# dyollb/segmantic

Hardware: AMD Instinct MI355X
Metric: 3D UNet train voxels/s on 128^3 bf16 (higher is better)
Workload: dtype bf16

## Files before the change

### include/segmi.h

```cpp
#ifndef SEGMI_H_
#define SEGMI_H_

#include <stddef.h>
#include <stdint.h>

#ifdef __cplusplus
extern "C" {
#endif

#define SEGMI_VERSION 1

enum { SEGMI_F32 = 0, SEGMI_BF16 = 1, SEGMI_F16 = 2 };
enum { SEGMI_OK = 0, SEGMI_EINVAL = -1, SEGMI_EUNSUPPORTED = -2, SEGMI_ELAUNCH = -3,
       SEGMI_EDATA = -4  };

typedef struct segmi_act {
  void* data;
  int32_t n, d, h, w;
  int32_t c;
  int32_t ld;
} segmi_act;

int segmi_version(void);
const char* segmi_last_error(void);
// ... 82 lines not shown
                               const void* packed, const float* bias, const float* prelu_alpha,
                               int act_channels, int ksize, int stride,
                               const float* bias_b , float* stats_partials ,
                               const segmi_bn_fin* stats_fin , void* stream);
int segmi_conv3d_fwd_pair(int dtype, const segmi_act* in, const segmi_act* out_a, const float* w_a,
                          const float* bias_a, const float* prelu_alpha_a, float* stats_partials_a,
                          const segmi_act* out_b, const float* w_b, const float* bias_b, int stride,
                          const segmi_bn_fin* stats_fin_a ,
                          const segmi_windows* windows ,
                          void* stream);

int segmi_convT3d_stats_rows(int dtype, const segmi_act* in, const segmi_act* out);
int segmi_convT3d_fwd(int dtype, const segmi_act* in, const segmi_act* out, const void* packed,
                      const float* w_src, const float* bias, const float* prelu_alpha,
                      const segmi_act* residual, float* stats_partials,
                      const segmi_bn_fin* stats_fin , void* stream);

int64_t segmi_conv3d_wgrad_workspace(int dtype, const segmi_act* x, const segmi_act* dy,
                                     int ksize, int stride, int cus);
int segmi_conv3d_wgrad(int dtype, const segmi_act* x, const segmi_act* dy, float* dw,
                       float* db, int ksize, int stride, void* workspace,
                       const segmi_in_affine* in_tf , int cus, void* stream);
int segmi_wgrad_cus(int cus);
int segmi_bias_grad(int dtype, const segmi_act* dy, float* db, void* workspace, void* stream);

int segmi_bn_stats_rows(const segmi_act* x);
int segmi_bn_stats(int dtype, const segmi_act* x, float* stats_partials, void* stream);
int segmi_bn_finalize(const float* stats_partials, int rows, int c, double count,
                      const float* gamma, const float* beta, float* running_mean,
                      float* running_var, float momentum, float eps, float* mean,
                      float* invstd, float* scale, float* shift, void* stream);
int segmi_bn_eval_affine(int c, const float* gamma, const float* beta,
                         const float* running_mean, const float* running_var, float eps,
                         float* scale, float* shift, void* stream);
int segmi_bn_act_fwd(int dtype, const segmi_act* x, const segmi_act* y, const float* scale,
                     const float* shift, const float* prelu_alpha, const segmi_act* residual,
                     float dropout_p, uint32_t dropout_seed, void* stream);
int segmi_bn_act_bwd_rows(const segmi_act* x);
int segmi_bn_act_bwd_reduce(int dtype, const segmi_act* dy, const segmi_act* x,
                            const float* mean, const float* invstd, const float* gamma,
                            const float* beta, const float* prelu_alpha, float* red_partials,
                            float dropout_p, uint32_t dropout_seed,
                            const segmi_bn_bwd_fin* fin , void* stream);
int segmi_bn_act_bwd_finalize(const float* red_partials, int rows, int c, double count,
                              const float* gamma, const float* invstd, float* dgamma,
                              float* dbeta, float* dalpha, float* coef, void* stream);
// ... 338 lines not shown
```

### segmantic_amd/_lib.py

```python
from __future__ import annotations

import ctypes as C
import os
from pathlib import Path

import torch

SEGMI_F32 = 0
SEGMI_BF16 = 1
SEGMI_F16 = 2

_LIB_PATH = Path(__file__).resolve().parent / "csrc" / "libsegmi.so"


class Act(C.Structure):

    _fields_ = [("data", C.c_void_p), ("n", C.c_int32), ("d", C.c_int32), ("h", C.c_int32),
                ("w", C.c_int32), ("c", C.c_int32), ("ld", C.c_int32)]


class WpackDesc(C.Structure):

    _fields_ = [("w_src", C.c_void_p), ("scale", C.c_void_p), ("packed", C.c_void_p),
                ("kind", C.c_int32), ("cin_k", C.c_int32), ("cout_k", C.c_int32),
# ... 50 lines not shown
    "segmi_last_error": (C.c_char_p, []),
    "segmi_stream_create_cumask": (_i, [_i, C.POINTER(C.c_void_p)]),
    "segmi_stream_destroy": (_i, [_P]),
    "segmi_wpack_bytes": (_i64, [_i, _i, _i, _i, _i]),
    "segmi_wpack": (_i, [_i, _i, _P, _P, _i, _i, _i, _P, _P]),
    "segmi_wpack_batch": (_i, [_i, C.POINTER(WpackDesc), _i, _P, _i, _P]),
    "segmi_conv3d_stats_rows": (_i, [_i, _AP, _AP, _i, _i]),
    "segmi_conv3d_in_affine_ok": (_i, [_i, _AP, _AP, _i, _i]),
    "segmi_conv3d_fwd_kernel_name": (C.c_char_p, [_i, _AP, _AP, _i, _i]),
    "segmi_conv3d_split_act_ok": (_i, [_i, _AP, _AP, _i, _i]),
    "segmi_conv3d_fwd_split_act": (_i, [_i, _AP, _AP, _P, _P, _P, _i, _i, _i, _P, _P, C.POINTER(BnFin), _P]),
    "segmi_conv3d_fwd": (_i, [_i, _AP, _AP, _P, _P, _i, _P, _P, _AP, _P, _i, _i, C.POINTER(InAffine),
                              C.POINTER(BnBwdSums), C.POINTER(BnFin), _P]),
    "segmi_conv3d_bn_bwd_sums_ok": (_i, [_i, _AP, _AP, _i, _i]),
    "segmi_dectop_ok": (_i, [_i, _AP, _AP]),
    "segmi_dectop_fwd": (_i, [_i, _AP, _AP, _P, _P, _P, _i, _P, _P, _P]),
    "segmi_conv3d_pair_ok": (_i, [_i, _AP, _AP, _AP]),
    "segmi_conv3d_fwd_pair": (_i, [_i, _AP, _AP, _P, _P, _P, _P, _AP, _P, _P, _i, C.POINTER(BnFin),
                                   C.POINTER(Windows), _P]),
    "segmi_convT3d_stats_rows": (_i, [_i, _AP, _AP]),
    "segmi_convT3d_fwd": (_i, [_i, _AP, _AP, _P, _P, _P, _P, _AP, _P, C.POINTER(BnFin), _P]),
    "segmi_conv3d_wgrad_workspace": (_i64, [_i, _AP, _AP, _i, _i, _i]),
    "segmi_conv3d_wgrad": (_i, [_i, _AP, _AP, _P, _P, _i, _i, _P, C.POINTER(InAffine), _i, _P]),
    "segmi_bias_grad": (_i, [_i, _AP, _P, _P, _P]),
    "segmi_bn_stats_rows": (_i, [_AP]),
    "segmi_bn_stats": (_i, [_i, _AP, _P, _P]),
    "segmi_bn_finalize": (_i, [_P, _i, _i, _d, _P, _P, _P, _P, _f, _f, _P, _P, _P, _P, _P]),
    "segmi_bn_eval_affine": (_i, [_i, _P, _P, _P, _P, _f, _P, _P, _P]),
    "segmi_bn_act_fwd": (_i, [_i, _AP, _AP, _P, _P, _P, _AP, _f, C.c_uint32, _P]),
    "segmi_bn_act_bwd_rows": (_i, [_AP]),
    "segmi_bn_act_bwd_reduce": (_i, [_i, _AP, _AP, _P, _P, _P, _P, _P, _P, _f, C.c_uint32,
                                     C.POINTER(BnBwdFin), _P]),
    "segmi_bn_act_bwd_finalize": (_i, [_P, _i, _i, _d, _P, _P, _P, _P, _P, _P, _P]),
    "segmi_bn_act_bwd_fused_ok": (_i, [_i, _AP, _AP, _AP]),
    "segmi_bn_act_bwd_fused_rows": (_i, [_AP]),
    "segmi_bn_act_bwd_fused": (_i, [_i, _AP, _AP, _AP, _P, _P, _P, _P, _P, _P, C.POINTER(BnBwdFin), _i, _P]),
    "segmi_bn_act_bwd_fused_wgs": (_i, [_i, _AP, _i]),
    "segmi_fused_timeouts": (C.c_uint, [_i]),
    "segmi_fused_test_hook": (_i, [C.c_uint, _i]),
    "segmi_bn_act_bwd_apply": (_i, [_i, _AP, _AP, _AP, _P, _P, _P, _P, _P, _P, _f, C.c_uint32, _P]),
    "segmi_bn_act_bwd_apply_conv_ok": (_i, [_i, _AP, _AP, _AP, _AP]),
    "segmi_bn_act_bwd_apply_conv": (_i, [_i, _AP, _AP, _AP, _P, _P, _P, _P, _P, _P, _AP, _P, _P]),
    "segmi_wgrad_cus": (_i, [_i]),
    "segmi_add": (_i, [_i, _AP, _AP, _AP, _P]),
    "segmi_cast_copy": (_i, [_i, _AP, _i, _AP, _P]),
    "segmi_nchw_to_ndhwc": (_i, [_P, _i, _AP, _P]),
# ... 151 lines not shown
```

### segmantic_amd/csrc/conv_small.hip

```cpp
#include "conv_shared.h"

namespace segmi {

struct SmallConvParams {
  const void* in;
  void* out;
  const float* w;
  const float* bias;
  const float* alpha;
  const void* res;
  float* stats;
  int N, Di, Hi, Wi, Do, Ho, Wo, Cout, ldi, ldo, ldr;
  int tz, ty, tx;
  void* out2;
  const float* w2;
  const float* bias2;
  int ldo2;
  int vec;
  int nwin;
  int wsy;
  int64_t wsz;
  int64_t woff[32];
  int fin_on;
  FinTail ft;
// ... 378 lines not shown
        }
      }
    }
  }

  __syncthreads();
  float* red = reinterpret_cast<float*>(smem);
#pragma unroll
  for (int nt = 0; nt < NTL; ++nt)
    *reinterpret_cast<f32x4*>(red + ((wave * NTL + nt) * 64 + lane) * 4) = acc[nt];
  __syncthreads();
  float* slab = p.partials + (int64_t)blockIdx.x * p.Cout * COMBOS;
  for (int o = tid; o < 16 * COMBOS; o += 256) {
    const int co = o / COMBOS, cb = o % COMBOS;
    const int nt = cb / 16, n16 = cb % 16;
    const int src = (nt * 64 + (co >> 2) * 16 + n16) * 4 + (co & 3);
    float sacc = 0.f;
#pragma unroll
    for (int w = 0; w < 4; ++w) sacc += red[w * NTL * 256 + src];
    slab[(int64_t)(co0 + co) * COMBOS + cb] = sacc;
  }
}

bool conv_small_ok(int cin, int cout, int ksize) {
  return ksize == 3 && cin >= 1 && cin <= 4 && (cout == 16 || cout == 32);
}

int conv_small_fwd_rows(const segmi_act* out) {
  return out->n * cdiv(out->d, 4) * cdiv(out->h, 8) * cdiv(out->w, 16);
}

template <typename T, int S, int CIN, bool PAIR>
static int launch_small_fwd_k(SmallConvParams p, hipStream_t st) {
  constexpr int HD = 3 * S + 3, HH = 7 * S + 3, HW = 15 * S + 3, XW = (HW + 6) / 4 * 4;
  constexpr int stage = CIN * HD * HH * XW * (int)sizeof(T);
  constexpr int lds0 = stage > 4 * 2 * 16 * 4 ? stage : 4 * 2 * 16 * 4;
  dim3 grid((unsigned)(p.N * p.tz * p.ty * p.tx), (unsigned)(p.Cout / 16));
  p.fin_on = p.fin_on && p.stats;
  const int lds = (int)fin_tail_arm(p, grid, 256, 2 * p.Cout, lds0);
  static int attr_set = 0;
  if (lds > 64 * 1024 && attr_set < lds) {
    (void)hipFuncSetAttribute((const void*)conv_small_fwd_kernel<T, S, CIN, PAIR>,
                              hipFuncAttributeMaxDynamicSharedMemorySize, lds);
    attr_set = lds;
  }
  hipLaunchKernelGGL((conv_small_fwd_kernel<T, S, CIN, PAIR>), grid, 256, lds, st, p);
// ... 62 lines not shown
  switch (cin) {
    case 1: return launch_small_wgrad<T, S, 1>(p, grid, st);
    case 2: return launch_small_wgrad<T, S, 2>(p, grid, st);
    case 3: return launch_small_wgrad<T, S, 3>(p, grid, st);
    default: return launch_small_wgrad<T, S, 4>(p, grid, st);
  }
}

int conv_small_wgrad(int dtype, const segmi_act* x, const segmi_act* dy, float* partials,
                     int stride, hipStream_t st) {
  SmallWgradParams p{};
  p.x = x->data; p.dy = dy->data; p.partials = partials;
  p.N = x->n; p.Dx = x->d; p.Hx = x->h; p.Wx = x->w; p.Dy = dy->d; p.Hy = dy->h; p.Wy = dy->w;
  p.Cout = dy->c; p.ldx = x->ld; p.ldy = dy->ld;
  p.tz = cdiv(dy->d, 2); p.ty = cdiv(dy->h, 8); p.tx = cdiv(dy->w, 16);
  p.ntiles = dy->n * p.tz * p.ty * p.tx;
  const int grid = conv_small_wgrad_slabs(dy);
#define SMALL_WGRAD(T) \
  return stride == 2 ? launch_small_wgrad_cin<T, 2>(p, x->c, grid, st) : launch_small_wgrad_cin<T, 1>(p, x->c, grid, st)
  SEGMI_BY_DTYPE(dtype, SMALL_WGRAD);
#undef SMALL_WGRAD
}

}
```

### segmantic_amd/csrc/wgrad.hip

```cpp
#include "wgrad_impl.h"
#include "reduce_fin.h"

#include <atomic>
namespace segmi {
static inline int clamp_cus(int n) {
  n = n / 8 * 8;
  return n < 8 ? 8 : (n > 256 ? 256 : n);
}
int wgrad_cus(int cus) {
  static const int env = [] {
    const char* e = getenv("SEGMI_WGRAD_CUS");
    return e ? clamp_cus(atoi(e)) : 0;
  }();
  if (env) return env;
  return cus > 0 ? clamp_cus(cus) : 256;
}
}
namespace segmi {

int wgrad_mfma_f32(const WgradParams& p, int ksize, int stride, int ct, int gx, hipStream_t st);
int wgrad_mfma_bf16(const WgradParams& p, int ksize, int stride, int ct, int gx, hipStream_t st);
int wgrad_mfma_f16(const WgradParams& p, int ksize, int stride, int ct, int gx, hipStream_t st);
int bn_stats_launch(int dtype, const segmi_act* x, float* partials, hipStream_t st, const BiasFin* bias_fin = nullptr);
int bn_stats_rows_for(const segmi_act* x);
bool conv_small_ok(int cin, int cout, int ksize);
int conv_small_wgrad_slabs(const segmi_act* dy);
int conv_small_wgrad(int dtype, const segmi_act* x, const segmi_act* dy, float* partials,
                     int stride, hipStream_t st);

struct WgDirectParams {
  const void* x;
  const void* dy;
  float* partials;
  int N, Dx, Hx, Wx, Dy, Hy, Wy, Cin, Cout, ldx, ldy, ks, stride;
  int64_t nvox;
  int chunk;
};

template <typename T>
__global__ __launch_bounds__(256) void wgrad_direct_kernel(WgDirectParams p) {
  const int nt = p.ks * p.ks * p.ks, pad = (p.ks - 1) / 2;
  const int nout = p.Cout * p.Cin * nt;
  const T* x = (const T*)p.x;
  const T* dy = (const T*)p.dy;
  for (int o = threadIdx.x; o < nout; o += 256) {
    const int tap = o % nt;
    const int ci = (o / nt) % p.Cin;
    const int co = o / (nt * p.Cin);
    const int kd = tap / (p.ks * p.ks), kh = (tap / p.ks) % p.ks, kw = tap % p.ks;
    float acc = 0.f;
    for (int64_t c0 = (int64_t)blockIdx.x * p.chunk; c0 < p.nvox; c0 += (int64_t)gridDim.x * p.chunk) {
      const int64_t c1 = c0 + p.chunk < p.nvox ? c0 + p.chunk : p.nvox;
      for (int64_t v = c0; v < c1; ++v) {
        int64_t t = v;
        const int ox = t % p.Wy; t /= p.Wy;
        const int oy = t % p.Hy; t /= p.Hy;
        const int oz = t % p.Dy;
        const int n = t / p.Dy;
        const int z = oz * p.stride - pad + kd, y = oy * p.stride - pad + kh,
                  xx = ox * p.stride - pad + kw;
        if ((unsigned)z >= (unsigned)p.Dx || (unsigned)y >= (unsigned)p.Hx ||
            (unsigned)xx >= (unsigned)p.Wx) continue;
        const float a = Elem<T>::ld(dy + v * p.ldy + co);
        const float b = Elem<T>::ld(x + ((((int64_t)n * p.Dx + z) * p.Hx + y) * p.Wx + xx) * p.ldx + ci);
        acc = fmaf(a, b, acc);
      }
    }
    p.partials[(int64_t)blockIdx.x * nout + o] = acc;
  }
}

constexpr int kSlabGroups = 16;
__global__ void slab_reduce_kernel(const float* __restrict__ partials, int nslab, int64_t n,
                                   float* __restrict__ out) {
  const int per = (nslab + gridDim.y - 1) / gridDim.y;
  const int b0 = blockIdx.y * per;
  const int b1 = b0 + per < nslab ? b0 + per : nslab;
  for (int64_t e = blockIdx.x * 256ll + threadIdx.x; e < n; e += (int64_t)gridDim.x * 256) {
    double a0 = 0.0, a1 = 0.0, a2 = 0.0, a3 = 0.0;
    int b = b0;
    for (; b + 3 < b1; b += 4) {
      a0 += (double)partials[(int64_t)b * n + e];
      a1 += (double)partials[(int64_t)(b + 1) * n + e];
      a2 += (double)partials[(int64_t)(b + 2) * n + e];
      a3 += (double)partials[(int64_t)(b + 3) * n + e];
    }
    for (; b < b1; ++b) a0 += (double)partials[(int64_t)b * n + e];
    out[(int64_t)blockIdx.y * n + e] = (float)((a0 + a1) + (a2 + a3));
  }
}

__global__ __launch_bounds__(1024) void slab_reduce_fused_kernel(const float* __restrict__ partials, int nslab,
                                                                 int64_t n, float* __restrict__ out) {
  __shared__ float gs[kSlabGroups][64];
  const int g = threadIdx.x >> 6, lane = threadIdx.x & 63;
  const int per = (nslab + kSlabGroups - 1) / kSlabGroups;
  const int b0 = g * per;
  const int b1 = b0 + per < nslab ? b0 + per : nslab;
  for (int64_t e0 = blockIdx.x * 64ll; e0 < n; e0 += (int64_t)gridDim.x * 64) {
    const int64_t e = e0 + lane;
    double a0 = 0.0, a1 = 0.0, a2 = 0.0, a3 = 0.0;
    if (e < n) {
      int b = b0;
      for (; b + 3 < b1; b += 4) {
        a0 += (double)partials[(int64_t)b * n + e];
        a1 += (double)partials[(int64_t)(b + 1) * n + e];
        a2 += (double)partials[(int64_t)(b + 2) * n + e];
        a3 += (double)partials[(int64_t)(b + 3) * n + e];
      }
      for (; b < b1; ++b) a0 += (double)partials[(int64_t)b * n + e];
    }
    gs[g][lane] = (float)((a0 + a1) + (a2 + a3));
    __syncthreads();
    if (g == 0 && e < n) {
      double c0 = 0.0, c1 = 0.0, c2 = 0.0, c3 = 0.0;
#pragma unroll
      for (int b = 0; b < kSlabGroups; b += 4) {
        c0 += (double)gs[b][lane];
        c1 += (double)gs[b + 1][lane];
        c2 += (double)gs[b + 2][lane];
        c3 += (double)gs[b + 3][lane];
      }
      out[e] = (float)((c0 + c1) + (c2 + c3));
    }
    __syncthreads();
  }
}


static inline bool aligned_rows(const segmi_act* a, int dtype) {
  const int es = dtype_size(dtype);
  return a->ld % (16 / es) == 0 && ((uintptr_t)a->data % 16) == 0;
}
static inline bool wg_mfma_ok(int dtype, const segmi_act* x, const segmi_act* dy, int ksize) {
  return x->c % 16 == 0 && dy->c % 16 == 0 && aligned_rows(x, dtype) && aligned_rows(dy, dtype) &&
         (ksize == 3 || ksize == 1);
}
static inline bool wg_small_ok(int dtype, const segmi_act* x, const segmi_act* dy, int ksize) {
  const int es = dtype_size(dtype);
  (void)es;
  return conv_small_ok(x->c, dy->c, ksize) && aligned_rows(dy, dtype);
}
static inline int wg_direct_blocks(const segmi_act* dy) {
  const int64_t b = cdiv64(act_voxels(dy), 512);
  return (int)(b > 1024 ? 1024 : b);
}
// ... 100 lines not shown
    p.nvox = act_voxels(dy); p.chunk = 512;
#define WG_DIRECT(T) hipLaunchKernelGGL(wgrad_direct_kernel<T>, slabs, 256, 0, st, p)
    SEGMI_BY_DTYPE(dtype, WG_DIRECT);
#undef WG_DIRECT
    SEGMI_LAUNCH_CHECK("conv3d_wgrad(direct)");
  }
  const int rb = grid_1d(nout, 2048);
  float* gsum = (float*)((char*)workspace + align256((int64_t)slabs * nout * 4));
  if (slabs > 2 * kSlabGroups) {
    const int fb = (int)(cdiv64(nout, 64) > 4096 ? 4096 : cdiv64(nout, 64));
    hipLaunchKernelGGL(slab_reduce_fused_kernel, dim3(fb), 1024, 0, st, (const float*)partials, slabs, nout, dw);
  } else {
    hipLaunchKernelGGL(slab_reduce_kernel, dim3(rb, 1), 256, 0, st, (const float*)partials, slabs,
                       nout, dw);
  }
  SEGMI_LAUNCH_CHECK("conv3d_wgrad(reduce)");
  if (db) {
    float* bws = (float*)((char*)gsum + align256((int64_t)kSlabGroups * nout * 4));
    return segmi_bias_grad(dtype, dy, db, bws, stream);
  }
  return SEGMI_OK;
}

}
```

### segmantic_amd/ops.py

```python
from __future__ import annotations

import ctypes as C
import math
from typing import Optional, Sequence

import numpy as np
import torch

from . import _lib
from ._lib import SEGMI_BF16, SEGMI_F16, SEGMI_F32, Act, BnBwdFin, BnBwdSums, BnFin, InAffine, Windows, check, lib

_DT = {torch.float32: SEGMI_F32, torch.bfloat16: SEGMI_BF16, torch.float16: SEGMI_F16}


def dtype_code(t: torch.Tensor) -> int:
    try:
        return _DT[t.dtype]
    except KeyError:
        raise TypeError(f"unsupported activation dtype {t.dtype} (float32 / bfloat16 / float16 only)")


def _stream() -> int:
    return torch.cuda.current_stream().cuda_stream

# ... 251 lines not shown
    return int(lib.segmi_convT3d_stats_rows(dtype_code(x), C.byref(ax), C.byref(ay)))


def convT3d_fwd(x, y, packed, w_src, bias, prelu_alpha=None, residual=None, stats=None,
                stats_fin=None) -> None:
    ax, ay = act(x), act(y)
    ar = act(residual) if residual is not None else None
    check(lib.segmi_convT3d_fwd(dtype_code(x), C.byref(ax), C.byref(ay), _ptr(packed),
                                _ptr(w_src), _ptr(bias), _ptr(prelu_alpha), _ref(ar),
                                _ptr(stats), _bn_fin(stats_fin), _stream()), "convT3d_fwd")


def conv3d_wgrad_workspace(x, dy, ksize, stride, cus: int = 0) -> int:
    ax, ay = act(x), act(dy)
    return int(lib.segmi_conv3d_wgrad_workspace(dtype_code(x), C.byref(ax), C.byref(ay), ksize,
                                                stride, int(cus)))


def conv3d_wgrad(x, dy, dw, db, ksize, stride, workspace, in_tf=None, cus: int = 0) -> None:
    ax, ay = act(x), act(dy)
    check(lib.segmi_conv3d_wgrad(dtype_code(x), C.byref(ax), C.byref(ay), _ptr(dw), _ptr(db),
                                 ksize, stride, _ptr(workspace), _in_affine(in_tf), int(cus), _stream()),
          "conv3d_wgrad")


def bias_grad(dy, db, workspace) -> None:
    ay = act(dy)
    check(lib.segmi_bias_grad(dtype_code(dy), C.byref(ay), _ptr(db), _ptr(workspace),
                              _stream()), "bias_grad")


def bn_stats_rows(x) -> int:
    ax = act(x)
    return int(lib.segmi_bn_stats_rows(C.byref(ax)))


def bn_stats(x, partials) -> None:
    ax = act(x)
    check(lib.segmi_bn_stats(dtype_code(x), C.byref(ax), _ptr(partials), _stream()), "bn_stats")


def bn_finalize(partials, rows, c, count, gamma, beta, running_mean, running_var, momentum,
                eps, mean, invstd, scale, shift) -> None:
    check(lib.segmi_bn_finalize(_ptr(partials), rows, c, float(count), _ptr(gamma), _ptr(beta),
                                _ptr(running_mean), _ptr(running_var), momentum, eps,
                                _ptr(mean), _ptr(invstd), _ptr(scale), _ptr(shift), _stream()),
# ... 1667 lines not shown
```

### segmantic_amd/seg/unet.py

```python
from __future__ import annotations

import math
import os
from typing import Dict, List, Optional, Sequence, Tuple

import torch
import torch.nn as nn

from .. import ops
from . import streams

_HALF = (torch.bfloat16, torch.float16)


class _Box(nn.Module):
    """Name-space node: holds children / parameters, computes nothing."""


def _conv_params(cin: int, cout: int, k: int, dims: int, transposed: bool) -> _Box:
    m = _Box()
    shape = ((cin, cout) if transposed else (cout, cin)) + (k,) * dims
    w = torch.empty(shape)
    nn.init.kaiming_uniform_(w, a=math.sqrt(5))
    fan_in = shape[1] * k ** dims
# ... 579 lines not shown
        if self._carry_open and conv in self._carry_convs:
            self._carried.append((conv, x, dy, need_bias, in_tf))
            return
        main = torch.cuda.current_stream()
        side = self._side_stream() if self.overlap_wgrad else None
        if side is not None:
            ev = torch.cuda.Event()
            ev.record(main)
            side.wait_event(ev)
        cus = self.wgrad_cus_overlap if side is not None else 0
        with torch.cuda.stream(side) if side is not None else _NullCtx():
            if conv.transposed:
                nbytes = ops.conv3d_wgrad_workspace(dy, x, 3, 2, cus)
                ws = self._scratch_buf("wgrad", nbytes)
                self._timed(conv.prefix + ":wgrad", ops.conv3d_wgrad, dy, x, conv.gw, None, 3, 2, ws, cus=cus)
                if need_bias:
                    ops.bias_grad(dy, conv.gb, ws)
            else:
                nbytes = ops.conv3d_wgrad_workspace(x, dy, conv.k, conv.stride, cus)
                ws = self._scratch_buf("wgrad", nbytes)
                self._timed(conv.prefix + ":wgrad", ops.conv3d_wgrad, x, dy, conv.gw,
                            conv.gb if need_bias else None, conv.k, conv.stride, ws, in_tf=in_tf, cus=cus)

    def _bsum_ok(self, conv: _Conv, dy, dx, bn: Optional["_BN"]) -> bool:
        return (bn is not None and self.fuse_bn_bwd and self.dtype in _HALF and self.dropout_p <= 0.0
                and not conv.transposed and conv.stride == 1 and conv.k == 3 and conv.mfma
                and conv.cout == 16
                and ops.conv3d_bn_bwd_sums_ok(dy, dx, 3, 1))

    def _dgrad(self, conv: _Conv, dy, dx, residual=None, bsum=None):
        if bsum is not None:
            bn, x_raw = bsum
            rows = ops.conv3d_stats_rows(dy, dx, conv.k, 1)
            part = self._fstat(rows, bn.c)
            self._timed(conv.prefix + ":dgrad", ops.conv3d_fwd, dy, dx, conv.dgrad_pack(), conv.w, 1,
                        None, conv.k, 1, residual=residual,
                        bn_bwd=(x_raw, bn.mean, bn.invstd, bn.gamma, bn.beta, bn.alpha, part),
                        bn_bwd_fin=self._bwd_fin(bn, x_raw))
            return rows
        if conv.transposed:
            ops.conv3d_fwd(dy, dx, conv.dgrad_pack(), conv.w, 0, None, 3, 2, residual=residual)
        elif conv.stride == 2:
            ops.convT3d_fwd(dy, dx, conv.dgrad_pack(), conv.w, None, residual=residual)
        else:
            self._timed(conv.prefix + ":dgrad", ops.conv3d_fwd, dy, dx, conv.dgrad_pack(), conv.w, 1,
                        None, conv.k, 1, residual=residual)
# ... 53 lines not shown
                self._timed(conv.prefix + ":fwd", ops.conv3d_fwd_split_act, x, m, conv.pair_pack(), conv.b, None,
                            conv.cout, conv.k, conv.stride, bias_b=ru["res"].b, stats=stats,
                            stats_fin=self._stats_fin(bn, r))
                saved[f"in{i}"] = cur
                saved[f"r{i}"] = r
                nconv = ru["units"][i + 1][0]
                if self._tf_ok(r, r, nconv) and nconv.cin == conv.cout and nconv.cout == conv.cout:
                    in_tf = (bn.scale, bn.shift, bn.alpha)
                    cur = r
                else:
                    a = self._buf(f"{pre}.a{i}", (n, d, h, w, conv.cout))
                    ops.bn_act_fwd(r, a, bn.scale, bn.shift, bn.alpha, dropout=bn.drop())
                    cur = a
                continue
            if i == 0 and paired:
                r = self._buf(f"{pre}.r{i}", (n, d, h, w, conv.cout))
                rows = ops.conv3d_stats_rows(x, r, conv.k, conv.stride)
                stats = self._fstat(rows, conv.cout)
                rc = ru["res"]
                self._timed(conv.prefix + ":fwd", ops.conv3d_fwd_pair, x, r, conv.w, conv.b, out,
                            rc.w, rc.b, conv.stride, stats_a=stats, stats_fin_a=self._stats_fin(bn, r))
                saved[f"in{i}"] = cur
                saved[f"r{i}"] = r
                nconv = ru["units"][i + 1][0]
                if self._tf_ok(r, r, nconv) and nconv.cin == conv.cout and nconv.cout == conv.cout:
                    in_tf = (bn.scale, bn.shift, bn.alpha)
                    cur = r
                else:
                    a = self._buf(f"{pre}.a{i}", (n, d, h, w, conv.cout))
                    ops.bn_act_fwd(r, a, bn.scale, bn.shift, bn.alpha, dropout=bn.drop())
                    cur = a
                continue
            if bn is None:
                self._timed(conv.prefix + ":fwd", ops.conv3d_fwd, cur, out, conv.fwd_pack(), conv.w,
                            0, conv.b, conv.k, conv.stride, residual=resid, in_tf=in_tf)
                saved[f"in{i}"] = cur
                saved[f"tf{i}"] = in_tf
                break
            r = self._buf(f"{pre}.r{i}", (n, d, h, w, conv.cout))
            self._conv_train(conv, cur, r, bn, in_tf=in_tf)
            saved[f"in{i}"] = cur
            saved[f"r{i}"] = r
            saved[f"tf{i}"] = in_tf
            in_tf = None
            if last:
                ops.bn_act_fwd(r, out, bn.scale, bn.shift, bn.alpha, residual=resid, dropout=bn.drop())
            else:
                nconv = ru["units"][i + 1][0]
                if self._tf_ok(r, r, nconv) and nconv.cin == conv.cout and nconv.cout == conv.cout:
                    in_tf = (bn.scale, bn.shift, bn.alpha)
                    cur = r
                else:
                    a = self._buf(f"{pre}.a{i}", (n, d, h, w, conv.cout))
                    ops.bn_act_fwd(r, a, bn.scale, bn.shift, bn.alpha, dropout=bn.drop())
                    cur = a
        self._saved[pre] = saved

    def _ru_bwd(self, ru, dout, dx=None, extra=None, dx_bn=None):
        pre = ru["prefix"]
        sv = self._saved[pre]
        x = sv["x"]
        nun = len(ru["units"])
        rc = ru["res"]
        if rc is not None and dx is not None:
            self._dgrad(rc, dout, dx, residual=extra)
        g = dout
        g_rows = 0
        for i in range(nun - 1, -1, -1):
            conv, bn = ru["units"][i]
            xin = sv[f"in{i}"]
            if bn is not None:
                r = sv[f"r{i}"]
                dr = self._buf(f"{pre}.dr{i}", r.shape)
                self._bn_bwd(bn, g, r, dr, sums_rows=g_rows)
            else:
                dr = g
            g_rows = 0
            self._wgrad(conv, xin, dr, need_bias=bn is None and conv is not self._top_bias_conv,
                        in_tf=sv.get(f"tf{i}"))
            if i > 0:
                da = self._buf(f"{pre}.da{i - 1}", xin.shape)
                pbn = ru["units"][i - 1][1]
                if self._bsum_ok(conv, dr, da, pbn):
                    g_rows = self._dgrad(conv, dr, da, bsum=(pbn, sv[f"r{i - 1}"]))
                else:
                    self._dgrad(conv, dr, da)
                g = da
            else:
                first_dr = dr
        if rc is not None:
            self._wgrad(rc, x, dout)
        self._grads_ready(self.param_offsets[f"model.{pre}.conv.unit0.conv.weight"][0])
        if dx is None:
            return 0
        conv0 = ru["units"][0][0]
        bsum = dx_bn if dx_bn is not None and self._bsum_ok(conv0, first_dr, dx, dx_bn[0]) else None
        if rc is not None:
            return self._dgrad(conv0, first_dr, dx, residual=dx, bsum=bsum) or 0
        if extra is not None:
            ops.add(dout, extra, dx)
            return self._dgrad(conv0, first_dr, dx, residual=dx, bsum=bsum) or 0
        return self._dgrad(conv0, first_dr, dx, residual=dout, bsum=bsum) or 0

    def _ru_fwd_eval(self, ru, x, out):
        pre = ru["prefix"]
        n, d, h, w = self._down_shape(x.shape, ru["stride"])
        paired = False
        merged = None
        if ru["res"] is not None:
            rc = ru["res"]
            paired = self._pair_ok(ru, x, out, f"{pre}.ea0", (n, d, h, w))
            if isinstance(x, ops.WindowBatch) and not paired:
                raise RuntimeError("window views need the first-layer pair kernel (window_views_ok said yes?)")
# ... 315 lines not shown
```

Before: 3.646 billion.

## Fuse first-unit BN backward apply with paired main and residual weight-gradient kernels

```diff
diff --git a/include/segmi.h b/include/segmi.h
--- a/include/segmi.h
+++ b/include/segmi.h
@@ -128,6 +128,14 @@
                        float* db, int ksize, int stride, void* workspace,
                        const segmi_in_affine* in_tf , int cus, void* stream);
 int segmi_wgrad_cus(int cus);
+int segmi_conv3d_wgrad_pair_ok(int dtype, const segmi_act* x, const segmi_act* g, const segmi_act* x_raw,
+                               const segmi_act* dy_b, int stride);
+int64_t segmi_conv3d_wgrad_pair_workspace(int dtype, const segmi_act* x, const segmi_act* dy_b);
+int segmi_conv3d_wgrad_pair(int dtype, const segmi_act* x, const segmi_act* g, const segmi_act* x_raw,
+                            const float* mean, const float* invstd, const float* gamma ,
+                            const float* beta , const float* prelu_alpha ,
+                            const float* coef, const segmi_act* dy_b, float* dw_a, float* dw_b,
+                            float* db_b , int stride, void* workspace, void* stream);
 int segmi_bias_grad(int dtype, const segmi_act* dy, float* db, void* workspace, void* stream);
 
 int segmi_bn_stats_rows(const segmi_act* x);
diff --git a/segmantic_amd/_lib.py b/segmantic_amd/_lib.py
--- a/segmantic_amd/_lib.py
+++ b/segmantic_amd/_lib.py
@@ -96,6 +96,9 @@
     "segmi_convT3d_fwd": (_i, [_i, _AP, _AP, _P, _P, _P, _P, _AP, _P, C.POINTER(BnFin), _P]),
     "segmi_conv3d_wgrad_workspace": (_i64, [_i, _AP, _AP, _i, _i, _i]),
     "segmi_conv3d_wgrad": (_i, [_i, _AP, _AP, _P, _P, _i, _i, _P, C.POINTER(InAffine), _i, _P]),
+    "segmi_conv3d_wgrad_pair_ok": (_i, [_i, _AP, _AP, _AP, _AP, _i]),
+    "segmi_conv3d_wgrad_pair_workspace": (_i64, [_i, _AP, _AP]),
+    "segmi_conv3d_wgrad_pair": (_i, [_i, _AP, _AP, _AP, _P, _P, _P, _P, _P, _P, _AP, _P, _P, _P, _i, _P, _P]),
     "segmi_bias_grad": (_i, [_i, _AP, _P, _P, _P]),
     "segmi_bn_stats_rows": (_i, [_AP]),
     "segmi_bn_stats": (_i, [_i, _AP, _P, _P]),
diff --git a/segmantic_amd/csrc/conv_small.hip b/segmantic_amd/csrc/conv_small.hip
--- a/segmantic_amd/csrc/conv_small.hip
+++ b/segmantic_amd/csrc/conv_small.hip
@@ -424,6 +424,206 @@
   }
 }
 
+struct SmallWgradPairParams {
+  const void* x;
+  const void* g;
+  const void* xraw;
+  const void* dyb;
+  const float* mean; const float* invstd; const float* gamma; const float* beta; const float* alpha;
+  const float* coef;
+  float* partials;
+  int N, Dx, Hx, Wx, Dy, Hy, Wy, Cout, ldx, ldg, ldr, ldyb;
+  int tz, ty, tx, ntiles;
+};
+
+template <typename T, int S, int CIN>
+__global__ __launch_bounds__(256) void conv_small_wgrad_pair_kernel(SmallWgradPairParams p) {
+  static_assert(sizeof(T) == 2, "16-bit storage");
+  constexpr int ES = 2;
+  constexpr int TD = 2, TH = 8, TW = 16, NV = TD * TH * TW, NL = NV / 16;
+  constexpr int HD = (TD - 1) * S + 3, HH = (TH - 1) * S + 3, HWX = (TW - 1) * S + 3;
+  constexpr int ROWS = HD * HH;
+  constexpr int YROWB = 16 * ES;
+  constexpr int COMBOS = 27 * CIN, NTL = (COMBOS + 15) / 16, CW = COMBOS + 1;
+  constexpr int NLY = NV * YROWB / 16 / 256;
+  constexpr int NXE = CIN * ROWS * HWX, NLX = (NXE + 255) / 256;
+  constexpr int XSE = CIN * 3 * ROWS * 16;
+  constexpr int ONES = ((TD - 1) * S * HH + (TH - 1) * S + 1) * 16;
+  static_assert(COMBOS < NTL * 16, "a spare column for the bias gradient");
+  static_assert(YROWB / 16 == 2 && NLY == 2, "a thread's channel chunk is tid % 2");
+  extern __shared__ __attribute__((aligned(16))) char smem[];
+  char* ysm = smem;
+  typedef typename RawOf<T>::type R;
+  R* xsm = reinterpret_cast<R*>(smem + 2 * NV * YROWB);
+  float* prm = reinterpret_cast<float*>(xsm + XSE + ONES);
+  const int tid = threadIdx.x, lane = tid & 63;
+  const int wave = __builtin_amdgcn_readfirstlane(tid >> 6);
+  const int g = lane >> 4, i16 = lane & 15;
+  const int co0 = blockIdx.y * 16;
+
+  int boff[NTL];
+#pragma unroll
+  for (int nt = 0; nt < NTL; ++nt) {
+    int cb = nt * 16 + i16;
+    const bool bias_col = cb == COMBOS;
+    if (cb > COMBOS - 1) cb = COMBOS - 1;
+    const int ci = cb / 27, tap = cb % 27;
+    const int kd = tap / 9, kh = (tap / 3) % 3, kw = tap % 3;
+    boff[nt] = bias_col ? XSE : ((ci * 3 + kw) * ROWS + kd * HH + kh) * 16;
+  }
+  const int ylane = (4 * g + (i16 >> 2)) * YROWB + 8 * (i16 & 3);
+
+  const bool has_alpha = p.alpha != nullptr;
+  const float alpha = has_alpha ? *p.alpha : 1.f;
+  if (tid < 96) {
+    const int which = tid >> 4, ch = co0 + (tid & 15);
+    prm[tid] = which == 0 ? p.mean[ch] : which == 1 ? p.invstd[ch] : which == 2 ? (p.gamma ? p.gamma[ch] : 1.f)
+             : which == 3 ? (p.beta ? p.beta[ch] : 0.f) : which == 4 ? p.coef[ch] : p.coef[p.Cout + ch];
+  }
+  for (int i = tid; i < ONES; i += 256) xsm[XSE + i] = (R)(H16<T>::pack2(1.f, 1.f) & 0xffffu);
+
+  f32x4 acc[NTL], accb[NTL];
+#pragma unroll
+  for (int nt = 0; nt < NTL; ++nt) acc[nt] = accb[nt] = f32x4{0.f, 0.f, 0.f, 0.f};
+
+  const R* x = (const R*)p.x;
+  const char* gb = (const char*)p.g;
+  const char* rb = (const char*)p.xraw;
+  const char* yb = (const char*)p.dyb;
+  frag_t ry[NLY], rr[NLY], rd[NLY];
+  unsigned yok = 0u;
+  R rx[NLX];
+  auto fetch = [&](int tile) {
+    int t = tile;
+    const int txi = t % p.tx; t /= p.tx;
+    const int tyi = t % p.ty; t /= p.ty;
+    const int tzi = t % p.tz;
+    const int n = t / p.tz;
+    const int oz0 = tzi * TD, oy0 = tyi * TH, ox0 = txi * TW;
+    yok = 0u;
+#pragma unroll
+    for (int k = 0; k < NLY; ++k) {
+      const int i = tid + 256 * k;
+      const int v = i / (YROWB / 16), ch = i % (YROWB / 16);
+      const int z = oz0 + v / (TW * TH), y = oy0 + (v / TW) % TH, xx = ox0 + v % TW;
+      ry[k] = rr[k] = rd[k] = frag_t{0u, 0u, 0u, 0u};
+      if (z < p.Dy && y < p.Hy && xx < p.Wy) {
+        const int64_t vox = (((int64_t)n * p.Dy + z) * p.Hy + y) * p.Wy + xx;
+        ry[k] = *reinterpret_cast<const frag_t*>(gb + (vox * p.ldg + co0) * ES + ch * 16);
+        rr[k] = *reinterpret_cast<const frag_t*>(rb + (vox * p.ldr + co0) * ES + ch * 16);
+        rd[k] = *reinterpret_cast<const frag_t*>(yb + (vox * p.ldyb + co0) * ES + ch * 16);
+        yok |= 1u << k;
+      }
+    }
+#pragma unroll
+    for (int k = 0; k < NLX; ++k) {
+      const int i = tid + 256 * k;
+      const int ci = i % CIN, r = i / CIN;
+      const int hx = r % HWX, hy = (r / HWX) % HH, hz = r / (HWX * HH);
+      const int z = oz0 * S - 1 + hz, y = oy0 * S - 1 + hy, xx = ox0 * S - 1 + hx;
+      rx[k] = (R)0;
+      if (i < NXE && (unsigned)z < (unsigned)p.Dx && (unsigned)y < (unsigned)p.Hx &&
+          (unsigned)xx < (unsigned)p.Wx)
+        rx[k] = x[((((int64_t)n * p.Dx + z) * p.Hx + y) * p.Wx + xx) * p.ldx + ci];
+    }
+  };
+  auto apply = [&](auto ha) {
+    constexpr bool HA = decltype(ha)::value;
+    const float* q8 = prm + 8 * (tid & 1);
+#pragma unroll
+    for (int q = 0; q < 4; ++q) {
+      const f32x2 m2 = *reinterpret_cast<const f32x2*>(q8 + 2 * q), i2 = *reinterpret_cast<const f32x2*>(q8 + 16 + 2 * q),
+                  g2 = *reinterpret_cast<const f32x2*>(q8 + 32 + 2 * q), b2 = *reinterpret_cast<const f32x2*>(q8 + 48 + 2 * q),
+                  c02 = *reinterpret_cast<const f32x2*>(q8 + 64 + 2 * q), c12 = *reinterpret_cast<const f32x2*>(q8 + 80 + 2 * q);
+#pragma unroll
+      for (int k = 0; k < NLY; ++k) {
+        const bool ok = (yok >> k) & 1u;
+        const f32x2 a{H16<T>::lo(rr[k][q]), H16<T>::hi(rr[k][q])};
+        const f32x2 d{H16<T>::lo(ry[k][q]), H16<T>::hi(ry[k][q])};
+        const f32x2 o2 = bn_bwd_apply_elem2<HA>(a, d, m2, i2, g2, b2, c02, c12, alpha);
+        ry[k][q] = ok ? H16<T>::pack2(o2[0], o2[1]) : 0u;
+      }
+    }
+  };
+  auto commit = [&]() {
+    if (has_alpha) apply(std::true_type{});
+    else apply(std::false_type{});
+#pragma unroll
+    for (int k = 0; k < NLY; ++k) {
+      *reinterpret_cast<frag_t*>(ysm + (tid + 256 * k) * 16) = ry[k];
+      *reinterpret_cast<frag_t*>(ysm + NV * YROWB + (tid + 256 * k) * 16) = rd[k];
+    }
+#pragma unroll
+    for (int k = 0; k < NLX; ++k) {
+      const int i = tid + 256 * k;
+      if (i >= NXE) continue;
+      const int ci = i % CIN, r = i / CIN;
+      const int hx = r % HWX, row = r / HWX;
+      R* pr = xsm + (ci * 3 * ROWS + row) * 16;
+#pragma unroll
+      for (int kw = 0; kw < 3; ++kw) {
+        const int d = hx - kw;
+        if (d >= 0 && d % S == 0 && d / S < 16) pr[kw * ROWS * 16 + d / S] = rx[k];
+      }
+    }
+  };
+
+  if ((int)blockIdx.x < p.ntiles) fetch(blockIdx.x);
+  for (int tile = blockIdx.x; tile < p.ntiles; tile += gridDim.x) {
+    __syncthreads();
+    commit();
+    __syncthreads();
+    if (tile + (int)gridDim.x < p.ntiles) fetch(tile + gridDim.x);
+#pragma unroll
+    for (int si = 0; si < NL / 2 / 4; ++si) {
+      const int s = wave + 4 * si;
+      const s16x4 lo = __builtin_amdgcn_ds_read_tr16_b64_v4i16(
+          (lds_s16x4*)(ysm + ylane + (2 * s) * 16 * YROWB));
+      const s16x4 hi = __builtin_amdgcn_ds_read_tr16_b64_v4i16(
+          (lds_s16x4*)(ysm + ylane + (2 * s + 1) * 16 * YROWB));
+      const s16x4 lob = __builtin_amdgcn_ds_read_tr16_b64_v4i16(
+          (lds_s16x4*)(ysm + NV * YROWB + ylane + (2 * s) * 16 * YROWB));
+      const s16x4 hib = __builtin_amdgcn_ds_read_tr16_b64_v4i16(
+          (lds_s16x4*)(ysm + NV * YROWB + ylane + (2 * s + 1) * 16 * YROWB));
+      const u32x2 l2 = __builtin_bit_cast(u32x2, lo), h2 = __builtin_bit_cast(u32x2, hi);
+      const u32x2 l2b = __builtin_bit_cast(u32x2, lob), h2b = __builtin_bit_cast(u32x2, hib);
+      const frag_t af = frag_t{l2[0], l2[1], h2[0], h2[1]};
+      const frag_t afb = frag_t{l2b[0], l2b[1], h2b[0], h2b[1]};
+      const int l0 = 2 * s, l1 = 2 * s + 1;
+      const int r0 = ((l0 / TH) * S * HH + (l0 % TH) * S) * 16 + 4 * g;
+      const int r1 = ((l1 / TH) * S * HH + (l1 % TH) * S) * 16 + 4 * g;
+#pragma unroll
+      for (int nt = 0; nt < NTL; ++nt) {
+        const u32x2 b0 = *reinterpret_cast<const u32x2*>(xsm + boff[nt] + r0);
+        const u32x2 b1 = *reinterpret_cast<const u32x2*>(xsm + boff[nt] + r1);
+        const frag_t bf = frag_t{b0[0], b0[1], b1[0], b1[1]};
+        acc[nt] = mma16<T>(af, bf, acc[nt]);
+        accb[nt] = mma16<T>(afb, bf, accb[nt]);
+      }
+    }
+  }
+
+  float* red = reinterpret_cast<float*>(smem);
+#pragma unroll
+  for (int half = 0; half < 2; ++half) {
+    __syncthreads();
+#pragma unroll
+    for (int nt = 0; nt < NTL; ++nt)
+      *reinterpret_cast<f32x4*>(red + ((wave * NTL + nt) * 64 + lane) * 4) = half ? accb[nt] : acc[nt];
+    __syncthreads();
+    float* slab = p.partials + ((int64_t)blockIdx.x * 2 + half) * p.Cout * CW;
+    for (int o = tid; o < 16 * CW; o += 256) {
+      const int co = o / CW, cb = o % CW;
+      const int nt = cb / 16, n16 = cb % 16;
+      const int src = (nt * 64 + (co >> 2) * 16 + n16) * 4 + (co & 3);
+      float sacc = 0.f;
+#pragma unroll
+      for (int w = 0; w < 4; ++w) sacc += red[w * NTL * 256 + src];
+      slab[(int64_t)(co0 + co) * CW + cb] = sacc;
+    }
+  }
+}
+
 bool conv_small_ok(int cin, int cout, int ksize) {
   return ksize == 3 && cin >= 1 && cin <= 4 && (cout == 16 || cout == 32);
 }
@@ -532,4 +732,51 @@
 #undef SMALL_WGRAD
 }
 
-}
+template <typename T, int S, int CIN>
+static int launch_small_wgrad_pair(const SmallWgradPairParams& p, int grid, hipStream_t st) {
+  if constexpr (sizeof(T) == 2) {
+    constexpr int HH = (8 - 1) * S + 3;
+    constexpr int ROWS = ((2 - 1) * S + 3) * HH;
+    constexpr int NTL = (27 * CIN + 15) / 16;
+    constexpr int ones = (S * HH + 7 * S + 1) * 16;
+    constexpr int stage = 2 * 256 * 16 * 2 + (CIN * 3 * ROWS * 16 + ones) * 2 + 6 * 16 * 4;
+    constexpr int red = 4 * NTL * 64 * 4 * 4;
+    constexpr int lds = stage > red ? stage : red;
+    return launch_wg256<conv_small_wgrad_pair_kernel<T, S, CIN>>(dim3(grid, p.Cout / 16), lds, lds > 64 * 1024, st,
+                                                                 "conv3d_wgrad_pair(small-cin)", p);
+  } else {
+    SEGMI_CHECK_ARG(false, "conv3d_wgrad_pair: 16-bit storage only (ask segmi_conv3d_wgrad_pair_ok first)");
+  }
+}
+
+template <typename T, int S>
+static int launch_small_wgrad_pair_cin(const SmallWgradPairParams& p, int cin, int grid, hipStream_t st) {
+  switch (cin) {
+    case 1: return launch_small_wgrad_pair<T, S, 1>(p, grid, st);
+    case 2: return launch_small_wgrad_pair<T, S, 2>(p, grid, st);
+    case 3: return launch_small_wgrad_pair<T, S, 3>(p, grid, st);
+    default: return launch_small_wgrad_pair<T, S, 4>(p, grid, st);
+  }
+}
+
+int conv_small_wgrad_pair(int dtype, const segmi_act* x, const segmi_act* g, const segmi_act* x_raw,
+                          const float* mean, const float* invstd, const float* gamma, const float* beta,
+                          const float* alpha, const float* coef, const segmi_act* dy_b, float* partials,
+                          int stride, hipStream_t st) {
+  SmallWgradPairParams p{};
+  p.x = x->data; p.g = g->data; p.xraw = x_raw->data; p.dyb = dy_b->data;
+  p.mean = mean; p.invstd = invstd; p.gamma = gamma; p.beta = beta; p.alpha = alpha; p.coef = coef;
+  p.partials = partials;
+  p.N = x->n; p.Dx = x->d; p.Hx = x->h; p.Wx = x->w; p.Dy = g->d; p.Hy = g->h; p.Wy = g->w;
+  p.Cout = g->c; p.ldx = x->ld; p.ldg = g->ld; p.ldr = x_raw->ld; p.ldyb = dy_b->ld;
+  p.tz = cdiv(g->d, 2); p.ty = cdiv(g->h, 8); p.tx = cdiv(g->w, 16);
+  p.ntiles = g->n * p.tz * p.ty * p.tx;
+  const int grid = conv_small_wgrad_slabs(g);
+#define SMALL_WGRAD_PAIR(T) \
+  return stride == 2 ? launch_small_wgrad_pair_cin<T, 2>(p, x->c, grid, st) \
+                     : launch_small_wgrad_pair_cin<T, 1>(p, x->c, grid, st)
+  SEGMI_BY_DTYPE(dtype, SMALL_WGRAD_PAIR);
+#undef SMALL_WGRAD_PAIR
+}
+
+}
diff --git a/segmantic_amd/csrc/wgrad.hip b/segmantic_amd/csrc/wgrad.hip
--- a/segmantic_amd/csrc/wgrad.hip
+++ b/segmantic_amd/csrc/wgrad.hip
@@ -27,6 +27,10 @@
 int conv_small_wgrad_slabs(const segmi_act* dy);
 int conv_small_wgrad(int dtype, const segmi_act* x, const segmi_act* dy, float* partials,
                      int stride, hipStream_t st);
+int conv_small_wgrad_pair(int dtype, const segmi_act* x, const segmi_act* g, const segmi_act* x_raw,
+                          const float* mean, const float* invstd, const float* gamma, const float* beta,
+                          const float* alpha, const float* coef, const segmi_act* dy_b, float* partials,
+                          int stride, hipStream_t st);
 
 struct WgDirectParams {
   const void* x;
@@ -71,25 +75,39 @@
 }
 
 constexpr int kSlabGroups = 16;
+__device__ __forceinline__ float slab_col_sum(const float* __restrict__ partials, int b0, int b1, int64_t n,
+                                              int64_t e) {
+  double a0 = 0.0, a1 = 0.0, a2 = 0.0, a3 = 0.0;
+  int b = b0;
+  for (; b + 3 < b1; b += 4) {
+    a0 += (double)partials[(int64_t)b * n + e];
+    a1 += (double)partials[(int64_t)(b + 1) * n + e];
+    a2 += (double)partials[(int64_t)(b + 2) * n + e];
+    a3 += (double)partials[(int64_t)(b + 3) * n + e];
+  }
+  for (; b < b1; ++b) a0 += (double)partials[(int64_t)b * n + e];
+  return (float)((a0 + a1) + (a2 + a3));
+}
 __global__ void slab_reduce_kernel(const float* __restrict__ partials, int nslab, int64_t n,
                                    float* __restrict__ out) {
   const int per = (nslab + gridDim.y - 1) / gridDim.y;
   const int b0 = blockIdx.y * per;
   const int b1 = b0 + per < nslab ? b0 + per : nslab;
-  for (int64_t e = blockIdx.x * 256ll + threadIdx.x; e < n; e += (int64_t)gridDim.x * 256) {
-    double a0 = 0.0, a1 = 0.0, a2 = 0.0, a3 = 0.0;
-    int b = b0;
-    for (; b + 3 < b1; b += 4) {
-      a0 += (double)partials[(int64_t)b * n + e];
-      a1 += (double)partials[(int64_t)(b + 1) * n + e];
-      a2 += (double)partials[(int64_t)(b + 2) * n + e];
-      a3 += (double)partials[(int64_t)(b + 3) * n + e];
-    }
-    for (; b < b1; ++b) a0 += (double)partials[(int64_t)b * n + e];
-    out[(int64_t)blockIdx.y * n + e] = (float)((a0 + a1) + (a2 + a3));
-  }
-}
-
+  for (int64_t e = blockIdx.x * 256ll + threadIdx.x; e < n; e += (int64_t)gridDim.x * 256)
+    out[(int64_t)blockIdx.y * n + e] = slab_col_sum(partials, b0, b1, n, e);
+}
+
+__device__ __forceinline__ float slab_groups_sum(const float (*gs)[64], int lane) {
+  double c0 = 0.0, c1 = 0.0, c2 = 0.0, c3 = 0.0;
+#pragma unroll
+  for (int b = 0; b < kSlabGroups; b += 4) {
+    c0 += (double)gs[b][lane];
+    c1 += (double)gs[b + 1][lane];
+    c2 += (double)gs[b + 2][lane];
+    c3 += (double)gs[b + 3][lane];
+  }
+  return (float)((c0 + c1) + (c2 + c3));
+}
 __global__ __launch_bounds__(1024) void slab_reduce_fused_kernel(const float* __restrict__ partials, int nslab,
                                                                  int64_t n, float* __restrict__ out) {
   __shared__ float gs[kSlabGroups][64];
@@ -99,29 +117,44 @@
   const int b1 = b0 + per < nslab ? b0 + per : nslab;
   for (int64_t e0 = blockIdx.x * 64ll; e0 < n; e0 += (int64_t)gridDim.x * 64) {
     const int64_t e = e0 + lane;
-    double a0 = 0.0, a1 = 0.0, a2 = 0.0, a3 = 0.0;
-    if (e < n) {
-      int b = b0;
-      for (; b + 3 < b1; b += 4) {
-        a0 += (double)partials[(int64_t)b * n + e];
-        a1 += (double)partials[(int64_t)(b + 1) * n + e];
-        a2 += (double)partials[(int64_t)(b + 2) * n + e];
-        a3 += (double)partials[(int64_t)(b + 3) * n + e];
-      }
-      for (; b < b1; ++b) a0 += (double)partials[(int64_t)b * n + e];
-    }
-    gs[g][lane] = (float)((a0 + a1) + (a2 + a3));
+    gs[g][lane] = e < n ? slab_col_sum(partials, b0, b1, n, e) : 0.f;
+    __syncthreads();
+    if (g == 0 && e < n) out[e] = slab_groups_sum(gs, lane);
+    __syncthreads();
+  }
+}
+
+struct PairDst {
+  float* dw_a; float* dw_b; float* db_b;
+  int cout, combos;
+  __device__ float* at(int64_t e) const {
+    const int row = (int)(e / (combos + 1)), cb = (int)(e % (combos + 1));
+    const bool b = row >= cout;
+    const int co = b ? row - cout : row;
+    if (cb < combos) return (b ? dw_b : dw_a) + (int64_t)co * combos + cb;
+    return b && db_b ? db_b + co : nullptr;
+  }
+};
+__global__ void slab_reduce_pair_kernel(const float* __restrict__ partials, int nslab, int64_t n, PairDst dst) {
+  for (int64_t e = blockIdx.x * 256ll + threadIdx.x; e < n; e += (int64_t)gridDim.x * 256) {
+    float* o = dst.at(e);
+    if (o) *o = slab_col_sum(partials, 0, nslab, n, e);
+  }
+}
+__global__ __launch_bounds__(1024) void slab_reduce_pair_fused_kernel(const float* __restrict__ partials, int nslab,
+                                                                      int64_t n, PairDst dst) {
+  __shared__ float gs[kSlabGroups][64];
+  const int g = threadIdx.x >> 6, lane = threadIdx.x & 63;
+  const int per = (nslab + kSlabGroups - 1) / kSlabGroups;
+  const int b0 = g * per;
+  const int b1 = b0 + per < nslab ? b0 + per : nslab;
+  for (int64_t e0 = blockIdx.x * 64ll; e0 < n; e0 += (int64_t)gridDim.x * 64) {
+    const int64_t e = e0 + lane;
+    gs[g][lane] = e < n ? slab_col_sum(partials, b0, b1, n, e) : 0.f;
     __syncthreads();
     if (g == 0 && e < n) {
-      double c0 = 0.0, c1 = 0.0, c2 = 0.0, c3 = 0.0;
-#pragma unroll
-      for (int b = 0; b < kSlabGroups; b += 4) {
-        c0 += (double)gs[b][lane];
-        c1 += (double)gs[b + 1][lane];
-        c2 += (double)gs[b + 2][lane];
-        c3 += (double)gs[b + 3][lane];
-      }
-      out[e] = (float)((c0 + c1) + (c2 + c3));
+      float* o = dst.at(e);
+      if (o) *o = slab_groups_sum(gs, lane);
     }
     __syncthreads();
   }
@@ -268,4 +301,49 @@
   return SEGMI_OK;
 }
 
-}
+int segmi_conv3d_wgrad_pair_ok(int dtype, const segmi_act* x, const segmi_act* g, const segmi_act* x_raw,
+                               const segmi_act* dy_b, int stride) {
+  if (!dtype_h16(dtype) || !act_ok(x) || !act_ok(g) || !act_ok(x_raw) || !act_ok(dy_b)) return 0;
+  if (stride != 1 && stride != 2) return 0;
+  for (const segmi_act* o : {x_raw, dy_b})
+    if (o->n != g->n || o->d != g->d || o->h != g->h || o->w != g->w || o->c != g->c) return 0;
+  if (x->n != g->n) return 0;
+  if (g->d != (x->d - 1) / stride + 1 || g->h != (x->h - 1) / stride + 1 || g->w != (x->w - 1) / stride + 1) return 0;
+  return conv_small_ok(x->c, g->c, 3) && aligned_rows(g, dtype) && aligned_rows(x_raw, dtype) &&
+         aligned_rows(dy_b, dtype);
+}
+
+int64_t segmi_conv3d_wgrad_pair_workspace(int dtype, const segmi_act* x, const segmi_act* dy_b) {
+  (void)dtype;
+  if (!x || !dy_b) return 0;
+  return align256((int64_t)conv_small_wgrad_slabs(dy_b) * 2 * dy_b->c * (27 * x->c + 1) * 4);
+}
+
+int segmi_conv3d_wgrad_pair(int dtype, const segmi_act* x, const segmi_act* g, const segmi_act* x_raw,
+                            const float* mean, const float* invstd, const float* gamma, const float* beta,
+                            const float* prelu_alpha, const float* coef, const segmi_act* dy_b, float* dw_a,
+                            float* dw_b, float* db_b, int stride, void* workspace, void* stream) {
+  SEGMI_CHECK_ARG(segmi_conv3d_wgrad_pair_ok(dtype, x, g, x_raw, dy_b, stride),
+                  "conv3d_wgrad_pair: not a 16-bit small-Cin k3 pair (ask segmi_conv3d_wgrad_pair_ok first)");
+  SEGMI_CHECK_ARG(mean && invstd && coef && dw_a && dw_b && workspace, "conv3d_wgrad_pair: bad arguments");
+  hipStream_t st = (hipStream_t)stream;
+  float* partials = (float*)workspace;
+  const int rc = conv_small_wgrad_pair(dtype, x, g, x_raw, mean, invstd, gamma, beta, prelu_alpha, coef, dy_b,
+                                       partials, stride, st);
+  if (rc) return rc;
+  const int slabs = conv_small_wgrad_slabs(dy_b);
+  const int combos = 27 * x->c;
+  const int64_t n = (int64_t)2 * g->c * (combos + 1);
+  const PairDst dst{dw_a, dw_b, db_b, g->c, combos};
+  if (slabs > 2 * kSlabGroups) {
+    hipLaunchKernelGGL(slab_reduce_pair_fused_kernel, dim3((unsigned)cdiv64(n, 64)), 1024, 0, st,
+                       (const float*)partials, slabs, n, dst);
+  } else {
+    hipLaunchKernelGGL(slab_reduce_pair_kernel, dim3(grid_1d(n, 2048)), 256, 0, st, (const float*)partials, slabs,
+                       n, dst);
+  }
+  SEGMI_LAUNCH_CHECK("conv3d_wgrad_pair(reduce)");
+  return SEGMI_OK;
+}
+
+}
diff --git a/segmantic_amd/ops.py b/segmantic_amd/ops.py
--- a/segmantic_amd/ops.py
+++ b/segmantic_amd/ops.py
@@ -297,6 +297,26 @@
     check(lib.segmi_conv3d_wgrad(dtype_code(x), C.byref(ax), C.byref(ay), _ptr(dw), _ptr(db),
                                  ksize, stride, _ptr(workspace), _in_affine(in_tf), int(cus), _stream()),
           "conv3d_wgrad")
+
+
+def conv3d_wgrad_pair_ok(x, g, x_raw, dy_b, stride) -> bool:
+    ax, ag, ar, ab = act(x), act(g), act(x_raw), act(dy_b)
+    return bool(lib.segmi_conv3d_wgrad_pair_ok(dtype_code(x), C.byref(ax), C.byref(ag), C.byref(ar),
+                                               C.byref(ab), stride))
+
+
+def conv3d_wgrad_pair_workspace(x, dy_b) -> int:
+    ax, ab = act(x), act(dy_b)
+    return int(lib.segmi_conv3d_wgrad_pair_workspace(dtype_code(x), C.byref(ax), C.byref(ab)))
+
+
+def conv3d_wgrad_pair(x, g, x_raw, mean, invstd, gamma, beta, prelu_alpha, coef, dy_b, dw_a, dw_b, db_b,
+                      stride, workspace) -> None:
+    ax, ag, ar, ab = act(x), act(g), act(x_raw), act(dy_b)
+    check(lib.segmi_conv3d_wgrad_pair(dtype_code(x), C.byref(ax), C.byref(ag), C.byref(ar), _ptr(mean),
+                                      _ptr(invstd), _ptr(gamma), _ptr(beta), _ptr(prelu_alpha), _ptr(coef),
+                                      C.byref(ab), _ptr(dw_a), _ptr(dw_b), _ptr(db_b), stride, _ptr(workspace),
+                                      _stream()), "conv3d_wgrad_pair")
 
 
 def bias_grad(dy, db, workspace) -> None:
diff --git a/segmantic_amd/seg/unet.py b/segmantic_amd/seg/unet.py
--- a/segmantic_amd/seg/unet.py
+++ b/segmantic_amd/seg/unet.py
@@ -625,6 +625,33 @@
                 self._timed(conv.prefix + ":wgrad", ops.conv3d_wgrad, x, dy, conv.gw,
                             conv.gb if need_bias else None, conv.k, conv.stride, ws, in_tf=in_tf, cus=cus)
 
+    fuse_first_wgrad = True
+
+    def _wgrad_pair_ok(self, ru, sv, g, g_rows: int, dout) -> bool:
+        units, rc = ru["units"], ru["res"]
+        conv, bn = units[0]
+        if not (self.fuse_first_wgrad and sv.get("paired") and rc is not None and bn is not None
+                and self.dtype in _HALF and self.dropout_p <= 0.0 and sv.get("tf0") is None):
+            return False
+        if self._carry_open and (conv in self._carry_convs or rc in self._carry_convs):
+            return False
+        r = sv["r0"]
+        if not g_rows and self.fuse_bn_bwd_small and ops.bn_act_bwd_fused_ok(g, r, r):
+            return False
+        return ops.conv3d_wgrad_pair_ok(sv["in0"], g, r, dout, conv.stride)
+
+    def _wgrad_pair(self, conv: _Conv, bn: "_BN", rc: _Conv, x, g, r, dout):
+        main = torch.cuda.current_stream()
+        side = self._side_stream() if self.overlap_wgrad else None
+        if side is not None:
+            ev = torch.cuda.Event()
+            ev.record(main)
+            side.wait_event(ev)
+        with torch.cuda.stream(side) if side is not None else _NullCtx():
+            ws = self._scratch_buf("wgrad", ops.conv3d_wgrad_pair_workspace(x, dout))
+            self._timed(conv.prefix + ":wgrad", ops.conv3d_wgrad_pair, x, g, r, bn.mean, bn.invstd, bn.gamma,
+                        bn.beta, bn.alpha, bn.coef, dout, conv.gw, rc.gw, rc.gb, conv.stride, ws)
+
     def _bsum_ok(self, conv: _Conv, dy, dx, bn: Optional["_BN"]) -> bool:
         return (bn is not None and self.fuse_bn_bwd and self.dtype in _HALF and self.dropout_p <= 0.0
                 and not conv.transposed and conv.stride == 1 and conv.k == 3 and conv.mfma
@@ -724,6 +751,7 @@
                             rc.w, rc.b, conv.stride, stats_a=stats, stats_fin_a=self._stats_fin(bn, r))
                 saved[f"in{i}"] = cur
                 saved[f"r{i}"] = r
+                saved["paired"] = True
                 nconv = ru["units"][i + 1][0]
                 if self._tf_ok(r, r, nconv) and nconv.cin == conv.cout and nconv.cout == conv.cout:
                     in_tf = (bn.scale, bn.shift, bn.alpha)
@@ -768,9 +796,19 @@
             self._dgrad(rc, dout, dx, residual=extra)
         g = dout
         g_rows = 0
+        pair_done = False
         for i in range(nun - 1, -1, -1):
             conv, bn = ru["units"][i]
             xin = sv[f"in{i}"]
+            if i == 0 and dx is None and self._wgrad_pair_ok(ru, sv, g, g_rows, dout):
+                r = sv["r0"]
+                if not g_rows:
+                    part = self._fstat(ops.bn_act_bwd_rows(r), bn.c)
+                    ops.bn_act_bwd_reduce(g, r, bn.mean, bn.invstd, bn.gamma, bn.beta, bn.alpha, part,
+                                          dropout=bn.drop(), fin=self._bwd_fin(bn, r))
+                self._wgrad_pair(conv, bn, rc, xin, g, r, dout)
+                pair_done = True
+                break
             if bn is not None:
                 r = sv[f"r{i}"]
                 dr = self._buf(f"{pre}.dr{i}", r.shape)
@@ -790,7 +828,7 @@
                 g = da
             else:
                 first_dr = dr
-        if rc is not None:
+        if rc is not None and not pair_done:
             self._wgrad(rc, x, dout)
         self._grads_ready(self.param_offsets[f"model.{pre}.conv.unit0.conv.weight"][0])
         if dx is None:
```

Measured after the change: 3.690 billion (median of 6 runs). 1.01x the previous value.
